# LiWentomng/OrientedRepPoints

Hardware: AMD Instinct MI355X
Metric: images/sec (1024x1024 DOTA, R-50 FPN) (higher is better)
Workload: dtype f32; 1 GPU; configs[1]: OrientedRepPoints R-50 FPN inference, 1024x1024 patch, 15 classes, bs=1/GPU, nms_pre=2000, score_thr=0.05, rnms iou_thr=0.4, max_per_img=2000; random-init weights, head biases calibrated to ~2000 dets/img; global_batch=1, parallelism=replicas x1 (image-parallel, no collective), images_in_flight_per_gpu=4

## Files before the change

include/orp_hip.h:

```cpp
#ifndef ORP_HIP_H_
#define ORP_HIP_H_

#include <stddef.h>
#include <stdint.h>

#ifdef __cplusplus
extern "C" {
#endif

#define ORP_OK 0
#define ORP_EINVAL (-1)
#define ORP_EWORKSPACE (-2)
#define ORP_ETOOBIG (-3)

const char* orp_version(void);

#define ORP_NMS_MAX_BOXES 131072
size_t orp_rnms_workspace_bytes(int n);
int orp_rnms(const float* dets, int n, float iou_thr, int flavor, int presorted, int order_out,
             int64_t* keep_out, int32_t* num_keep, void* workspace, size_t workspace_bytes, void* stream);

size_t orp_rnms_batched_workspace_bytes(int n_total, int nseg, int max_seg);
int orp_rnms_batched(const float* dets, int n_total, const int32_t* seg_offsets, int nseg, int max_seg,
                     float iou_thr, int flavor, int64_t* keep_out, int32_t* num_keep,
// ... 236 lines not shown
int orp_conv1x1_pack_weight(const float* weight, int c_out, int c_in, float* packed, void* stream);
int orp_conv1x1_multi(const orp_bias_level* levels_host, int nlevels, int batch, int c_in, int c_out,
                      const float* weight_packed, const float* bias, const float* sub, int relu, void* stream);

int orp_conv1x1_bn_act_ok(int c_in, int c_out);
int orp_conv1x1_bn_act_pays(int c_in, int c_out, int hw, int batch, int has_residual);
int orp_conv1x1_bn_act_tile(int c_in, int c_out, int hw, int batch, int* tile_channels, int* tile_positions);
int orp_conv1x1_bn_act(const float* x, const float* weight_t, const float* scale, const float* shift, const float* residual,
                       const float* scale2, const float* shift2, float* y, int batch, int c_in, int c_out, int hw, int relu,
                       void* stream);

int orp_conv1x1_bn_act_range(const float* x, const float* weight_t, const float* scale, const float* shift, const float* residual,
                             const float* scale2, const float* shift2, float* y, int batch, int c_in, int c_out, int hw, int relu,
                             uint32_t* range_out, void* stream);
int orp_conv1x1_bn_act_pieces_ok(int c_in, int c_out);
int orp_conv1x1_bn_act_pieces_pays(int c_in, int c_out, int hw, int batch, int has_residual);
int orp_conv1x1_bn_act_pieces_tile(int c_in, int c_out, int hw, int batch, int* tile_channels, int* tile_positions);
size_t orp_conv1x1_bn_pieces_packed_bytes(int c_in, int c_out);
int orp_conv1x1_bn_pieces_pack_weight(const float* weight, int c_in, int c_out, void* packed, void* stream);
int orp_conv1x1_bn_act_pieces(const float* x, const void* weight_packed, const float* scale, const float* shift,
                              const float* residual, const float* scale2, const float* shift2, float* y, int batch, int c_in,
                              int c_out, int hw, int relu, uint32_t* range_out, void* stream);

int orp_affine_act_range(const float* x, const float* residual, const float* scale, const float* shift, float* y, int batch,
                         int channels, int hw, int relu, uint32_t* range_out, void* stream);

int orp_conv3x3_bn_act_ok(int c_in, int c_out);
int orp_conv3x3_bn_act_pays(int c_in, int c_out, int height, int width, int batch);
int orp_conv3x3_bn_act_tile(int c_in, int c_out, int height, int width, int batch, int* tile_h, int* tile_w, int* waves_pos,
                            int* waves_ch);
size_t orp_conv3x3_bn_packed_bytes(int c_in, int c_out);
int orp_conv3x3_bn_pack_weight(const float* weight, int c_in, int c_out, void* packed, void* stream);
int orp_conv3x3_bn_act(const float* x, const void* weight_packed, const float* scale, const float* shift, const uint32_t* range_in,
                       float* y, int batch, int c_in, int c_out, int height, int width, int relu, void* stream);


int orp_conv3x3_small_ok(int c_in, int c_out);
int orp_conv3x3_small_multi(const orp_norm_level* levels_host, int nlevels, int batch, int c_in, int c_out,
                            const float* weight_packed, void* stream);
int orp_conv3x3_small_multi_ex(const orp_norm_level* levels_host, const float* const* weights_packed_host, int nlevels,
                               int batch, int c_in, int c_out, void* stream);
size_t orp_conv3x3_small_workspace_bytes(const orp_norm_level* levels_host, const int* strides_host, int nlevels, int batch,
                                         int c_out);
int orp_conv3x3_small_multi_strided(const orp_norm_level* levels_host, const float* const* weights_packed_host,
                                    const int* strides_host, int nlevels, int batch, int c_in, int c_out, void* workspace,
                                    size_t workspace_bytes, void* stream);
// ... 72 lines not shown
```

orientedreppoints_amd/_lib.py:

```python
import ctypes
import os

import torch

_HERE = os.path.dirname(os.path.abspath(__file__))
LIB_PATH = os.environ.get("ORP_HIP_LIB") or os.path.join(_HERE, "csrc", "liborp_hip.so")

ORP_OK, ORP_EINVAL, ORP_EWORKSPACE, ORP_ETOOBIG = 0, -1, -2, -3
ORP_NMS_MAX_BOXES = 131072

_vp = ctypes.c_void_p
_i = ctypes.c_int
_f = ctypes.c_float
_sz = ctypes.c_size_t

_SIGNATURES = {
    "orp_version": (ctypes.c_char_p, []),
    "orp_rnms_workspace_bytes": (_sz, [_i]),
    "orp_rnms": (_i, [_vp, _i, _f, _i, _i, _i, _vp, _vp, _vp, _sz, _vp]),
    "orp_rnms_batched_workspace_bytes": (_sz, [_i, _i, _i]),
    "orp_rnms_batched": (_i, [_vp, _i, _vp, _i, _i, _f, _i, _vp, _vp, _vp, _sz, _vp]),
    "_poly_nms": (None, [_vp, _vp, _vp, _i, _i, _f, _i]),
    "_overlaps": (None, [_vp, _vp, _vp, _i, _i, _i]),
    "orp_quad_iou_matrix": (_i, [_vp, _i, _vp, _i, _i, _i, _vp, _vp]),
# ... 63 lines not shown
                                     _i, _vp, _vp]),
    "orp_scene_tiles_flip": (_i, [_vp, _i, _i, ctypes.c_longlong, _vp, _i, _i, _vp, _vp, _i, _i, _vp, _vp]),
    "orp_scene_tiles_resized_flip": (_i, [_vp, _i, _i, ctypes.c_longlong, _vp, _i, _i, _i, _i, _i, _i, _i, _vp, _vp, _vp, _vp, _vp,
                                          _vp, _i, _i, _vp, _vp]),
    "orp_scene_collect_workspace_bytes": (_sz, [_i, _i]),
    "orp_scene_collect": (_i, [_vp, _i, _i, _vp, ctypes.c_double, _i, _i, _vp, _vp, _vp, _vp, _vp, _sz, _vp]),
    "orp_soft_rnms_host": (_i, [_vp, _i, _f, _i, _f, _f, _vp, _vp]),
    "orp_conv1x1_packed_floats": (_sz, [_i]),
    "orp_conv1x1_ok": (_i, [_i, _i]),
    "orp_conv1x1_pack_weight": (_i, [_vp, _i, _i, _vp, _vp]),
    "orp_conv1x1_multi": (_i, [_vp, _i, _i, _i, _i, _vp, _vp, _vp, _i, _vp]),
    "orp_conv1x1_bn_act_ok": (_i, [_i, _i]),
    "orp_conv1x1_bn_act_pays": (_i, [_i, _i, _i, _i, _i]),
    "orp_conv1x1_bn_act_tile": (_i, [_i, _i, _i, _i, _vp, _vp]),
    "orp_conv1x1_bn_act": (_i, [_vp, _vp, _vp, _vp, _vp, _vp, _vp, _vp, _i, _i, _i, _i, _i, _vp]),
    "orp_conv1x1_bn_act_range": (_i, [_vp, _vp, _vp, _vp, _vp, _vp, _vp, _vp, _i, _i, _i, _i, _i, _vp, _vp]),
    "orp_affine_act_range": (_i, [_vp, _vp, _vp, _vp, _vp, _i, _i, _i, _i, _vp, _vp]),
    "orp_conv1x1_bn_act_pieces_ok": (_i, [_i, _i]),
    "orp_conv1x1_bn_act_pieces_pays": (_i, [_i, _i, _i, _i, _i]),
    "orp_conv1x1_bn_act_pieces_tile": (_i, [_i, _i, _i, _i, _vp, _vp]),
    "orp_conv1x1_bn_pieces_packed_bytes": (_sz, [_i, _i]),
    "orp_conv1x1_bn_pieces_pack_weight": (_i, [_vp, _i, _i, _vp, _vp]),
    "orp_conv1x1_bn_act_pieces": (_i, [_vp, _vp, _vp, _vp, _vp, _vp, _vp, _vp, _i, _i, _i, _i, _i, _vp, _vp]),
    "orp_conv3x3_bn_act_ok": (_i, [_i, _i]),
    "orp_conv3x3_bn_act_pays": (_i, [_i, _i, _i, _i, _i]),
    "orp_conv3x3_bn_act_tile": (_i, [_i, _i, _i, _i, _i, _vp, _vp, _vp, _vp]),
    "orp_conv3x3_bn_packed_bytes": (_sz, [_i, _i]),
    "orp_conv3x3_bn_pack_weight": (_i, [_vp, _i, _i, _vp, _vp]),
    "orp_conv3x3_bn_act": (_i, [_vp, _vp, _vp, _vp, _vp, _vp, _i, _i, _i, _i, _i, _i, _vp]),
    "orp_pp_select_scratch_bytes": (_sz, [_i, _i, _i]),
    "orp_pp_select": (_i, [_vp, _i, _i, _vp, _i, _i, _vp, _vp, _sz, _vp]),
    "orp_pp_gather": (_i, [_vp, _vp, _i, _i, _vp, _vp, _vp, _i, _vp, _vp, _vp, _vp, _vp]),
    "orp_pp_compact_scratch_bytes": (_sz, [_i]),
    "orp_pp_compact": (_i, [_vp, _vp, _i, _i, _i, _vp, _f, _i, _vp, _vp, _vp, _vp, _vp, _vp, _sz, _vp]),
    "orp_pp_compact_views_scratch_bytes": (_sz, [_i]),
    "orp_pp_compact_views": (_i, [_vp, _i, _i, _f, _i, _vp, _vp, _vp, _vp, _vp, _vp, _vp, _vp, _sz, _vp]),
    "orp_pp_pack": (_i, [_vp, _vp, _vp, _vp, _vp, _vp, _vp, _vp, _i, _i, _vp, _vp]),
    "orp_groupnorm_workspace_bytes": (_sz, [_vp, _i, _i, _i, _i]),
    "orp_groupnorm_act_multi": (_i, [_vp, _i, _i, _i, _i, _vp, _vp, _f, _i, _vp, _sz, _vp]),
    "orp_groupnorm_act_multi_ex": (_i, [_vp, _vp, _vp, _i, _i, _i, _i, _f, _i, _vp, _sz, _vp]),
    "orp_groupnorm_act_multi_nhwc": (_i, [_vp, _vp, _vp, _vp, _i, _i, _i, _i, _f, _i, _vp, _sz, _vp]),
    "orp_groupnorm_act_multi_train": (_i, [_vp, _vp, _vp, _i, _i, _i, _i, _f, _i, _vp, _vp, _sz, _vp]),
    "orp_groupnorm_backward_workspace_bytes": (_sz, [_vp, _i, _i, _i, _i]),
    "orp_groupnorm_act_multi_backward": (_i, [_vp, _vp, _vp, _vp, _vp, _vp, _vp, _i, _i, _i, _i, _i, _vp, _vp, _sz, _vp]),
    "orp_voc_best_match_f64": (_i, [_vp, _vp, _i, _vp, _vp, _i, _vp, _vp, _vp]),
    "orp_affine_act": (_i, [_vp, _vp, _vp, _vp, _vp, _i, _i, _i, _i, _vp]),
# ... 104 lines not shown
```

orientedreppoints_amd/csrc/orp_conv1x1_bn_pieces.hip:

```cpp
#include <hip/hip_runtime.h>
#include <stdint.h>

#include "../../include/orp_hip.h"
#include "orp_affine.hpp"
#include "orp_range.hpp"
#include "orp_launch.hpp"

namespace {

constexpr int kThreads = 256;

typedef float f32x16 __attribute__((ext_vector_type(16)));
typedef __bf16 bf8 __attribute__((ext_vector_type(8)));

struct Args {
  const float* x;
  const uint16_t* planes;
  size_t plane_stride;
  const float* scale; const float* shift;
  const float* res;
  const float* scale2; const float* shift2;
  float* y;
  int cin, cout, hw, relu;
  int ntm, ntn;
  unsigned* range;
};

__global__ void pack_pieces_kernel(const float* __restrict__ w, int cout, int cin, uint16_t* __restrict__ planes) {
  const long total = (long)cout * cin;
  for (long i = (long)blockIdx.x * blockDim.x + threadIdx.x; i < total; i += (long)gridDim.x * blockDim.x) {
    const int e = (int)(i & 7);
    long r = i >> 3;
    const int o = (int)(r % cout); r /= cout;
    const int kg = (int)(r & 1);
    const int cblk = (int)(r >> 1);
    const int c = cblk * 16 + kg * 8 + e;
    const float v = w[(long)o * cin + c];
    const float v0 = __uint_as_float(__float_as_uint(v) & 0xffff0000u);
    const float r1 = v - v0;
    const float v1 = __uint_as_float(__float_as_uint(r1) & 0xffff0000u);
    const float v2 = r1 - v1;
    planes[i] = (uint16_t)(__float_as_uint(v0) >> 16);
    planes[total + i] = (uint16_t)(__float_as_uint(v1) >> 16);
    planes[2 * total + i] = (uint16_t)(__float_as_uint(v2) >> 16);
  }
}

__device__ __forceinline__ unsigned pack_hi16(float a, float b) {
  return __builtin_amdgcn_perm(__float_as_uint(b), __float_as_uint(a), 0x07060302u);
}

__device__ __forceinline__ void split_pair(float a, float b, unsigned (&d)[3]) {
  const float a0 = __uint_as_float(__float_as_uint(a) & 0xffff0000u), b0 = __uint_as_float(__float_as_uint(b) & 0xffff0000u);
  const float ar = a - a0, br = b - b0;
  const float a1 = __uint_as_float(__float_as_uint(ar) & 0xffff0000u), b1 = __uint_as_float(__float_as_uint(br) & 0xffff0000u);
  d[0] = pack_hi16(a0, b0);
  d[1] = pack_hi16(a1, b1);
  d[2] = pack_hi16(ar - a1, br - b1);
}

template <int WCH, int WN, int BK, bool VEC, int MODE, bool RANGE = false>
__global__ void __launch_bounds__(kThreads, 2)
conv1x1_bn_pieces_kernel(const Args P) {
  constexpr int ASTR = BK + 8;
  constexpr int NCH = BK / 16;
  constexpr int WPOS = 4 / WCH;
  constexpr int BM = 32 * WCH, BN = 32 * WN * WPOS;
  constexpr int PLANE = BN * ASTR, BUF = 3 * PLANE;
  constexpr int ITEMS = (BK / 2) * (BN / 4);
  constexpr int XV = (ITEMS + kThreads - 1) / kThreads;
  __shared__ __align__(16) uint16_t lds[2 * BUF + 8 * BM];
  float* Cs = reinterpret_cast<float*>(lds + 2 * BUF);

  const int tid = threadIdx.x;
  const int bid = blockIdx.x;
  const int mt = bid % P.ntm, rest = bid / P.ntm;
  const int nt = rest % P.ntn, b = rest / P.ntn;
  const int m0 = mt * BM, p0 = nt * BN;
  const int hw = P.hw, cout = P.cout;
  const float* xb = P.x + (size_t)b * P.cin * hw;
  if (tid < BM) {
    const int ch = min(m0 + tid, cout - 1);
    Cs[tid] = P.scale[ch]; Cs[BM + tid] = P.shift[ch];
    if (MODE == 2) { Cs[2 * BM + tid] = P.scale2[ch]; Cs[3 * BM + tid] = P.shift2[ch]; }
  }

  const int lane = tid & 63, wave = tid >> 6;
  const int kg = lane >> 5, l31 = lane & 31;
  const int wm0 = (wave / WPOS) * 32, wn0 = (wave % WPOS) * 32 * WN;

  const uint16_t* wp = P.planes + ((size_t)kg * cout + min(m0 + wm0 + l31, cout - 1)) * 8;
  const size_t wblk = (size_t)2 * cout * 8;
  bf8 wq[NCH][3];
  auto load_w = [&](int t, int c) {
    const uint16_t* a = wp + (size_t)(t * NCH + c) * wblk;
#pragma unroll
    for (int pl = 0; pl < 3; pl++) wq[c][pl] = *reinterpret_cast<const bf8*>(a + (size_t)pl * P.plane_stride);
  };
#pragma unroll
  for (int c = 0; c < NCH; c++) load_w(0, c);

  float4 xr[2][XV][2];
  int xpq[XV], xkp[XV];
#pragma unroll
  for (int i = 0; i < XV; i++) {
    const int idx = tid + i * kThreads;
    if (BN >= 64) {
      const int r = idx >> 5;
      xpq[i] = (idx & 15) + 16 * (r % (BN / 64));
      xkp[i] = ((idx >> 4) & 1) + 2 * (r / (BN / 64));
    } else {
      xpq[i] = idx & (BN / 4 - 1);
      xkp[i] = idx / (BN / 4);
    }
    xkp[i] &= BK / 2 - 1;
  }
  auto fetch = [&](int k0, float4 (&xr)[XV][2]) {
#pragma unroll
    for (int i = 0; i < XV; i++) {
      const int col = p0 + 4 * xpq[i];
#pragma unroll
      for (int h = 0; h < 2; h++) {
        const float* src = xb + (size_t)(k0 + 2 * xkp[i] + h) * hw;
        if (VEC) {
          xr[i][h] = *reinterpret_cast<const float4*>(src + min(col, hw - 4));
        } else {
          xr[i][h].x = src[min(col, hw - 1)]; xr[i][h].y = src[min(col + 1, hw - 1)];
          xr[i][h].z = src[min(col + 2, hw - 1)]; xr[i][h].w = src[min(col + 3, hw - 1)];
        }
      }
    }
  };
  auto stage = [&](int buf, const float4 (&xr)[XV][2]) {
#pragma unroll
    for (int i = 0; i < XV; i++) {
      if (ITEMS % kThreads != 0 && tid + i * kThreads >= ITEMS) continue;
      const int col = p0 + 4 * xpq[i];
      float v[2][4];
#pragma unroll
      for (int h = 0; h < 2; h++) {
        v[h][0] = col < hw ? xr[i][h].x : 0.f; v[h][1] = col + 1 < hw ? xr[i][h].y : 0.f;
        v[h][2] = col + 2 < hw ? xr[i][h].z : 0.f; v[h][3] = col + 3 < hw ? xr[i][h].w : 0.f;
      }
      const int rot = (xpq[i] >> 1) & 3;
#pragma unroll
      for (int h = 0; h < 2; h++) {
        if (rot & 1) { const float t0 = v[h][0]; v[h][0] = v[h][1]; v[h][1] = v[h][2]; v[h][2] = v[h][3]; v[h][3] = t0; }
        if (rot & 2) { const float t0 = v[h][0], t1 = v[h][1]; v[h][0] = v[h][2]; v[h][1] = v[h][3]; v[h][2] = t0; v[h][3] = t1; }
      }
      unsigned* base = reinterpret_cast<unsigned*>(lds + buf * BUF) + xkp[i];
#pragma unroll
      for (int j = 0; j < 4; j++) {
        unsigned d[3];
        split_pair(v[0][j], v[1][j], d);
        unsigned* dst = base + (4 * xpq[i] + ((j + rot) & 3)) * (ASTR / 2);
#pragma unroll
        for (int pl = 0; pl < 3; pl++) dst[pl * (PLANE / 2)] = d[pl];
      }
    }
  };

  f32x16 acc[WN];
#pragma unroll
  for (int ni = 0; ni < WN; ni++)
#pragma unroll
    for (int r = 0; r < 16; r++) acc[ni][r] = 0.f;

  auto mma = [&](int buf, int t_next) {
    const uint16_t* xa = lds + buf * BUF + (wn0 + l31) * ASTR + 8 * kg;
    auto load_x = [&](int c, bf8 (&q)[WN][3]) {
#pragma unroll
      for (int ni = 0; ni < WN; ni++)
#pragma unroll
        for (int pl = 0; pl < 3; pl++) q[ni][pl] = *reinterpret_cast<const bf8*>(xa + pl * PLANE + ni * 32 * ASTR + c * 16);
    };
    constexpr bool AHEAD = WN <= 2;
    bf8 xqs[AHEAD ? 2 : 1][WN][3];
    load_x(0, xqs[0]);
#pragma unroll
    for (int c = 0; c < NCH; c++) {
      bf8 (&xq)[WN][3] = xqs[AHEAD ? (c & 1) : 0];
      if (AHEAD) { if (c + 1 < NCH) load_x(c + 1, xqs[(c + 1) & 1]); }
      else if (c > 0) load_x(c, xqs[0]);
      __builtin_amdgcn_sched_barrier(0);
#pragma unroll
      for (int ni = 0; ni < WN; ni++) acc[ni] = __builtin_amdgcn_mfma_f32_32x32x16_bf16(wq[c][0], xq[ni][2], acc[ni], 0, 0, 0);
#pragma unroll
      for (int ni = 0; ni < WN; ni++) acc[ni] = __builtin_amdgcn_mfma_f32_32x32x16_bf16(wq[c][2], xq[ni][0], acc[ni], 0, 0, 0);
#pragma unroll
      for (int ni = 0; ni < WN; ni++) acc[ni] = __builtin_amdgcn_mfma_f32_32x32x16_bf16(wq[c][1], xq[ni][1], acc[ni], 0, 0, 0);
#pragma unroll
      for (int ni = 0; ni < WN; ni++) acc[ni] = __builtin_amdgcn_mfma_f32_32x32x16_bf16(wq[c][0], xq[ni][1], acc[ni], 0, 0, 0);
#pragma unroll
      for (int ni = 0; ni < WN; ni++) acc[ni] = __builtin_amdgcn_mfma_f32_32x32x16_bf16(wq[c][1], xq[ni][0], acc[ni], 0, 0, 0);
#pragma unroll
      for (int ni = 0; ni < WN; ni++) acc[ni] = __builtin_amdgcn_mfma_f32_32x32x16_bf16(wq[c][0], xq[ni][0], acc[ni], 0, 0, 0);
      __builtin_amdgcn_sched_barrier(0);
      load_w(t_next, c);
      __builtin_amdgcn_sched_barrier(0);
    }
  };

  const int nk = P.cin / BK;
  auto step = [&](int t, float4 (&cur)[XV][2], float4 (&nxt)[XV][2], int buf) {
    fetch(min(t + 2, nk - 1) * BK, cur);
    __builtin_amdgcn_sched_barrier(0);
    mma(buf, t + 1);
    stage(buf ^ 1, nxt);
    __syncthreads();
  };
  fetch(0, xr[0]);
  stage(0, xr[0]);
  fetch(min(1, nk - 1) * BK, xr[1]);
  __syncthreads();
  int t = 0;
  for (; t + 2 < nk; t += 2) {
    step(t, xr[0], xr[1], 0);
    step(t + 1, xr[1], xr[0], 1);
  }
  if (t + 1 < nk) step(t, xr[0], xr[1], 0);

  const size_t plane0 = (size_t)b * cout;
  float rv[WN][16];
  if (MODE) {
#pragma unroll
    for (int ni = 0; ni < WN; ni++) {
      const int p = min(p0 + wn0 + 32 * ni + l31, hw - 1);
#pragma unroll
      for (int r = 0; r < 16; r++) {
        const int ch = min(m0 + wm0 + 8 * (r >> 2) + 4 * kg + (r & 3), cout - 1);
        rv[ni][r] = P.res[(plane0 + ch) * hw + p];
      }
    }
  }
  __builtin_amdgcn_sched_barrier(0);
  mma((nk - 1) & 1, nk - 1);

  unsigned rmax = 0u;
#pragma unroll
  for (int g = 0; g < 4; g++) {
    const int chg = m0 + wm0 + 8 * g + 4 * kg;
    const float* cs = Cs + wm0 + 8 * g + 4 * kg;
    const float4 a4 = *reinterpret_cast<const float4*>(cs);
    const float4 b4 = *reinterpret_cast<const float4*>(cs + BM);
    const float av[4] = {a4.x, a4.y, a4.z, a4.w}, bv[4] = {b4.x, b4.y, b4.z, b4.w};
    float a2v[4] = {0.f, 0.f, 0.f, 0.f}, b2v[4] = {0.f, 0.f, 0.f, 0.f};
    if (MODE == 2) {
      const float4 c4 = *reinterpret_cast<const float4*>(cs + 2 * BM);
      const float4 d4 = *reinterpret_cast<const float4*>(cs + 3 * BM);
      a2v[0] = c4.x; a2v[1] = c4.y; a2v[2] = c4.z; a2v[3] = c4.w;
      b2v[0] = d4.x; b2v[1] = d4.y; b2v[2] = d4.z; b2v[3] = d4.w;
    }
#pragma unroll
    for (int ni = 0; ni < WN; ni++) {
      const int p = p0 + wn0 + 32 * ni + l31;
#pragma unroll
      for (int q = 0; q < 4; q++) {
        const int r = 4 * g + q;
        const float v = acc[ni][r];
        float t;
        if (MODE == 0) t = affine_act(v, av[q], bv[q], P.relu);
        else if (MODE == 1) t = affine_res_act(v, av[q], bv[q], rv[ni][r], P.relu);
        else t = affine_res_act(v, av[q], bv[q], affine_act(rv[ni][r], a2v[q], b2v[q], 0), P.relu);
        if (chg < cout && p < hw) {
          P.y[(plane0 + chg + q) * hw + p] = t;
          if (RANGE) rmax = max(rmax, orp::range_bits(t));
        }
      }
    }
  }
  if (RANGE) {
#pragma unroll
    for (int o = 32; o > 0; o >>= 1) rmax = max(rmax, (unsigned)__shfl_xor((int)rmax, o, 64));
    unsigned* red = reinterpret_cast<unsigned*>(lds);
    __syncthreads();
    if (lane == 0) red[wave] = rmax;
    __syncthreads();
    if (tid == 0) orp::range_raise(P.range, max(max(red[0], red[1]), max(red[2], red[3])));
  }
}

struct Tile { int bm, bn; };

Tile pick_tile(int cout, int hw, int batch) {
  if (cout <= 64) return Tile{64, 128};
// ... 1 lines not shown
  for (int i = 0; i < 3; i++) {
    const Tile t = cand[i];
    const long wgs = (long)((cout + t.bm - 1) / t.bm) * ((hw + t.bn - 1) / t.bn) * batch;
    if (wgs >= 512) return t;
  }
  return cand[2];
}

template <int WCH, int WN, int BK, int MODE>
void launch_mode(const Args& A, int batch, bool vec, hipStream_t st) {
  const dim3 grid((unsigned)((long)A.ntm * A.ntn * batch));
  if (vec) hipLaunchKernelGGL((conv1x1_bn_pieces_kernel<WCH, WN, BK, true, MODE>), grid, dim3(kThreads), 0, st, A);
  else hipLaunchKernelGGL((conv1x1_bn_pieces_kernel<WCH, WN, BK, false, MODE>), grid, dim3(kThreads), 0, st, A);
}
template <int WCH, int WN, int BK>
void launch(const Args& A, int batch, bool vec, hipStream_t st) {
  if (A.range) {
    const dim3 grid((unsigned)((long)A.ntm * A.ntn * batch));
    if (vec) hipLaunchKernelGGL((conv1x1_bn_pieces_kernel<WCH, WN, BK, true, 0, true>), grid, dim3(kThreads), 0, st, A);
    else hipLaunchKernelGGL((conv1x1_bn_pieces_kernel<WCH, WN, BK, false, 0, true>), grid, dim3(kThreads), 0, st, A);
  } else if (!A.res) launch_mode<WCH, WN, BK, 0>(A, batch, vec, st);
  else if (!A.scale2) launch_mode<WCH, WN, BK, 1>(A, batch, vec, st);
  else launch_mode<WCH, WN, BK, 2>(A, batch, vec, st);
}

}

extern "C" {

int orp_conv1x1_bn_act_pieces_ok(int c_in, int c_out) {
  return (c_in >= 64 && c_in <= 2048 && c_in % 64 == 0 && c_out >= 64 && c_out <= 4096 && c_out % 32 == 0) ? 1 : 0;
}

int orp_conv1x1_bn_act_pieces_tile(int c_in, int c_out, int hw, int batch, int* tile_channels, int* tile_positions) {
  if (!orp_conv1x1_bn_act_pieces_ok(c_in, c_out) || hw <= 0 || batch <= 0) return 0;
  const Tile t = pick_tile(c_out, hw, batch);
  if (tile_channels) *tile_channels = t.bm;
  if (tile_positions) *tile_positions = t.bn;
  return 1;
}

int orp_conv1x1_bn_act_pieces_pays(int c_in, int c_out, int hw, int batch, int has_residual) {
  if (!orp_conv1x1_bn_act_pieces_ok(c_in, c_out) || hw <= 0 || batch <= 0) return 0;
  (void)has_residual;
  static const struct { int cin, cout, hw_min, hw_max, batch; } paid[] = {
      {64, 64, 65536, 65536, 1},
      {256, 64, 65536, 147456, 1},  {256, 64, 65536, 65536, 2},
      {64, 256, 65536, 147456, 1},  {64, 256, 65536, 65536, 2},
      {256, 128, 65536, 147456, 1}, {256, 128, 65536, 65536, 2},
      {512, 128, 16384, 36864, 1},  {512, 128, 16384, 16384, 2},
      {128, 512, 16384, 36864, 1},  {128, 512, 16384, 16384, 2},
      {512, 256, 16384, 36864, 1},  {512, 256, 16384, 16384, 2},
      {1024, 256, 4096, 9216, 1},   {1024, 256, 4096, 4096, 2},
      {256, 1024, 4096, 9216, 1},   {256, 1024, 4096, 4096, 2},
      {1024, 512, 4096, 9216, 1},   {1024, 512, 4096, 4096, 2},
      {2048, 512, 2304, 2304, 1},   {2048, 512, 1024, 1024, 2},
      {512, 2048, 1024, 2304, 1},   {512, 2048, 1024, 1024, 2},
  };
  for (const auto& s : paid)
    if (s.cin == c_in && s.cout == c_out && s.batch == batch && hw >= s.hw_min && hw <= s.hw_max) return 1;
  return 0;
}

size_t orp_conv1x1_bn_pieces_packed_bytes(int c_in, int c_out) {
  return orp_conv1x1_bn_act_pieces_ok(c_in, c_out) ? (size_t)6 * c_in * c_out : 0;
}

int orp_conv1x1_bn_pieces_pack_weight(const float* weight, int c_in, int c_out, void* packed, void* stream) {
  if (!weight || !packed || ((uintptr_t)packed & 15) || !orp_conv1x1_bn_act_pieces_ok(c_in, c_out)) return ORP_EINVAL;
  const long total = (long)c_in * c_out;
  const int blocks = (int)((total + 255) / 256 < 4096 ? (total + 255) / 256 : 4096);
  hipLaunchKernelGGL(pack_pieces_kernel, dim3(blocks), dim3(256), 0, (hipStream_t)stream, weight, c_out, c_in,
                     reinterpret_cast<uint16_t*>(packed));
  hipError_t e = hipGetLastError();
  return e == hipSuccess ? ORP_OK : (int)e;
}

int orp_conv1x1_bn_act_pieces(const float* x, const void* weight_packed, const float* scale, const float* shift, const float* residual,
                              const float* scale2, const float* shift2, float* y, int batch, int c_in, int c_out, int hw, int relu,
                              uint32_t* range_out, void* stream) {
  if (range_out && residual) return ORP_EINVAL;
  if (!x || !weight_packed || !scale || !shift || !y || batch <= 0 || hw <= 0 || !orp_conv1x1_bn_act_pieces_ok(c_in, c_out))
    return ORP_EINVAL;
// ... 2 lines not shown
  if ((uintptr_t)weight_packed & 15) return ORP_EINVAL;
  const Tile t = pick_tile(c_out, hw, batch);
  Args A;
  A.x = x; A.planes = reinterpret_cast<const uint16_t*>(weight_packed); A.plane_stride = (size_t)c_in * c_out;
  A.scale = scale; A.shift = shift; A.res = residual; A.scale2 = scale2; A.shift2 = shift2; A.y = y;
  A.cin = c_in; A.cout = c_out; A.hw = hw; A.relu = relu ? 1 : 0;
  A.ntm = (c_out + t.bm - 1) / t.bm; A.ntn = (hw + t.bn - 1) / t.bn;
  A.range = range_out;
  if ((long)A.ntm * A.ntn * batch >= (1L << 31)) return ORP_ETOOBIG;
  const bool vec = (hw & 3) == 0 && ((uintptr_t)x & 15) == 0;
  hipStream_t st = (hipStream_t)stream;
  if (range_out) {
    hipError_t fe = orp::fill_async(range_out, 0, sizeof(uint32_t), st);
    if (fe != hipSuccess) return (int)fe;
  }
  if (t.bm == 64) launch<2, 2, 32>(A, batch, vec, st);
  else if (t.bn == 128) launch<4, 4, 32>(A, batch, vec, st);
  else if (t.bn == 64) launch<4, 2, 64>(A, batch, vec, st);
  else launch<4, 1, 64>(A, batch, vec, st);
  hipError_t e = hipGetLastError();
  return e == hipSuccess ? ORP_OK : (int)e;
}

}
```

orientedreppoints_amd/mmdet_models/resnet.py:

```python
import torch
import torch.nn as nn

from .layers import build_conv_layer, build_norm_layer, constant_init, kaiming_init
from .registry import BACKBONES


class Bottleneck(nn.Module):
    expansion = 4

    def __init__(self, inplanes, planes, stride=1, dilation=1, downsample=None, style='pytorch',
                 norm_cfg=dict(type='BN'), dcn=None):
        super(Bottleneck, self).__init__()
        assert style in ['pytorch', 'caffe']
        assert dcn is None or isinstance(dcn, dict)
        if style == 'pytorch':
            conv1_stride, conv2_stride = 1, stride
        else:
            conv1_stride, conv2_stride = stride, 1
        self.conv1 = nn.Conv2d(inplanes, planes, kernel_size=1, stride=conv1_stride, bias=False)
        self.add_module('bn1', build_norm_layer(norm_cfg, planes)[1])
        self.with_dcn = dcn is not None
        fallback_on_stride = False
        if self.with_dcn:
            fallback_on_stride = dcn.pop('fallback_on_stride', False)
            dcn = dict(dcn)
            if 'modulated' in dcn:
                dcn.setdefault('type', 'DCNv2' if dcn.pop('modulated') else 'DCN')
            dcn.setdefault('type', 'DCN')
        use_dcn = self.with_dcn and not fallback_on_stride
        self.conv2 = build_conv_layer(dcn if use_dcn else None, planes, planes, kernel_size=3, stride=conv2_stride,
                                      padding=dilation, dilation=dilation, bias=False)
        self.conv2_is_dcn = use_dcn
        self.add_module('bn2', build_norm_layer(norm_cfg, planes)[1])
        self.conv3 = nn.Conv2d(planes, planes * self.expansion, kernel_size=1, bias=False)
        self.add_module('bn3', build_norm_layer(norm_cfg, planes * self.expansion)[1])
        self.relu = nn.ReLU(inplace=True)
        self.downsample = downsample

    def _fused_ok(self, x):
        return (not torch.is_grad_enabled()) and x.is_cuda and x.dtype == torch.float32 and \
            isinstance(self.bn1, nn.BatchNorm2d) and not self.bn1.training and not self.bn3.training

    def _downsample_norm_fusable(self):
        from .. import switches
        on = getattr(self, 'fuse_downsample_norm', None)
        if on is None:
            on = switches.BN_DOWNSAMPLE_FUSE
        ds = self.downsample
        return bool(on) and isinstance(ds, nn.Sequential) and len(ds) == 2 and isinstance(ds[0], nn.Conv2d) and \
            isinstance(ds[1], nn.BatchNorm2d) and not ds[1].training

    def _conv1x1_fusable(self):
        from .. import switches
        on = getattr(self, 'fuse_conv1x1', None)
        if on is None:
            on = switches.BN_CONV1X1_FUSE
        return bool(on)

    def _conv1x1_pieces_on(self):
        from .. import switches
        on = getattr(self, 'fuse_conv1x1_pieces', None)
        if on is None:
            on = switches.BN_CONV1X1_PIECES
        return bool(on)

    def _conv3x3_fusable(self):
        from .. import switches
        on = getattr(self, 'fuse_conv3x3', None)
        if on is None:
            on = switches.BN_CONV3X3_FUSE
        return bool(on) and not self.conv2_is_dcn and isinstance(self.bn2, nn.BatchNorm2d) and not self.bn2.training

    def _forward_fused(self, x):
        from ..mmdet_ops.fused_norm import bn_act, conv1x1_bn_act, conv3x3_bn_act, conv3x3_bn_act_routed
        fuse = self._conv1x1_fusable()
        pieces = None if self._conv1x1_pieces_on() else False

        def conv_bn_act(t, conv, bn, **kw):
            if fuse:
                return conv1x1_bn_act(t, conv, bn, pieces=pieces, **kw)
            return bn_act(conv(t).contiguous(), bn, **kw)
        force3 = bool(getattr(self, 'force_conv3x3', False))
        fuse3 = False
        if self._conv3x3_fusable() and tuple(self.conv1.stride) == (1, 1):
            fuse3 = conv3x3_bn_act_routed(x, self.conv2, self.bn2, force3,
                                          shape=(x.size(0), self.conv1.out_channels, x.size(2), x.size(3)))
        if fuse3:
            out, bits = conv_bn_act(x, self.conv1, self.bn1, relu=True, want_range=True)
            out = conv3x3_bn_act(out, self.conv2, self.bn2, relu=True, force=force3, range_bits=bits)
        else:
            out = conv_bn_act(x, self.conv1, self.bn1, relu=True)
            out = bn_act(self.conv2(out).contiguous(), self.bn2, relu=True)
        if self._downsample_norm_fusable():
            return conv_bn_act(out, self.conv3, self.bn3, residual=self.downsample[0](x).contiguous(),
                               residual_bn=self.downsample[1], relu=True)
        if self.downsample is not None:
            identity = bn_act(self.downsample[0](x).contiguous(), self.downsample[1], relu=False)
        else:
            identity = x.contiguous()
        return conv_bn_act(out, self.conv3, self.bn3, residual=identity, relu=True)

    def forward(self, x):
        if self._fused_ok(x):
            return self._forward_fused(x)
        identity = x
        out = self.relu(self.bn1(self.conv1(x)))
        out = self.relu(self.bn2(self.conv2(out)))
        out = self.bn3(self.conv3(out))
        if self.downsample is not None:
            identity = self.downsample(x)
        out += identity
        return self.relu(out)


@BACKBONES.register_module
# ... 130 lines not shown
```

orientedreppoints_amd/mmdet_ops/fused_norm.py:

```python
import ctypes

import torch

from .. import _lib, _packcache


class _NormLevel(ctypes.Structure):
    _fields_ = [("input", ctypes.c_void_p), ("output", ctypes.c_void_p), ("height", ctypes.c_int),
                ("width", ctypes.c_int)]


def _norm_levels(ins, outs):
    levels = (_NormLevel * len(ins))()
    for i, (x, y) in enumerate(zip(ins, outs)):
        levels[i] = _NormLevel(x.data_ptr(), y.data_ptr() if y is not None else None, x.size(2), x.size(3))
    return levels


def _gn_modules(gn, n, who):
    gns = list(gn) if isinstance(gn, (list, tuple)) else [gn] * n
    if len(gns) != n or any(g.num_groups != gns[0].num_groups or g.eps != gns[0].eps for g in gns):
        raise ValueError(who + ": one GroupNorm per tensor, equal num_groups / eps")
    index, distinct, owner = {}, [], []
    for g in gns:
# ... 232 lines not shown
    if residual is not None:
        residual = residual.detach()
        if not (tuple(residual.shape) == (B, cout, H, W) and residual.is_contiguous() and residual.dtype == torch.float32):
            raise ValueError("conv1x1_bn_act: residual must be a contiguous fp32 tensor of the output's shape")
    wt = _transposed_1x1_weight(conv.weight)
    scale, shift = _bn_affine(bn)
    scale2, shift2 = _bn_affine(residual_bn) if residual_bn is not None else (None, None)
    y = torch.empty((B, cout, H, W), dtype=torch.float32, device=x.device)
    if want_range:
        bits = torch.empty(1, dtype=torch.int32, device=x.device)
        with torch.cuda.device(x.device):
            rc = L.orp_conv1x1_bn_act_range(_lib.ptr(x), _lib.ptr(wt), _lib.ptr(scale), _lib.ptr(shift), None, None, None,
                                            _lib.ptr(y), B, cin, cout, H * W, 1 if relu else 0, _lib.ptr(bits), _lib.stream_of(x))
        _lib.check(rc, "orp_conv1x1_bn_act_range")
        return y, bits
    with torch.cuda.device(x.device):
        rc = L.orp_conv1x1_bn_act(_lib.ptr(x), _lib.ptr(wt), _lib.ptr(scale), _lib.ptr(shift), _lib.ptr(residual),
                                  _lib.ptr(scale2), _lib.ptr(shift2), _lib.ptr(y), B, cin, cout, H * W, 1 if relu else 0,
                                  _lib.stream_of(x))
    _lib.check(rc, "orp_conv1x1_bn_act")
    return y


def conv3x3_bn_act_ok(x, conv, bn, shape=None):
    w = getattr(conv, 'weight', None)
    shape = tuple(x.shape) if shape is None else tuple(shape)
    return bool(type(conv) is torch.nn.Conv2d and isinstance(bn, torch.nn.BatchNorm2d) and not bn.training and
                x.is_cuda and x.dtype == torch.float32 and len(shape) == 4 and w.dtype == torch.float32 and w.dim() == 4 and
                w.size(2) == 3 and w.size(3) == 3 and shape[1] == w.size(1) and conv.bias is None and
                tuple(conv.stride) == (1, 1) and tuple(conv.padding) == (1, 1) and tuple(conv.dilation) == (1, 1) and
                conv.groups == 1 and shape[0] * shape[2] * shape[3] > 0 and _lib.lib().orp_conv3x3_bn_act_ok(w.size(1), w.size(0)))


def conv3x3_bn_act_routed(x, conv, bn, force=False, shape=None):
    if not conv3x3_bn_act_ok(x, conv, bn, shape):
        return False
    B, _c, H, W = tuple(x.shape) if shape is None else tuple(shape)
    return bool(force or _lib.lib().orp_conv3x3_bn_act_pays(conv.weight.size(1), conv.weight.size(0), H, W, B))


def conv3x3_bn_act_tile(cin, cout, H, W, B):
    v = [ctypes.c_int() for _ in range(4)]
    if not _lib.lib().orp_conv3x3_bn_act_tile(int(cin), int(cout), int(H), int(W), int(B), *[ctypes.byref(t) for t in v]):
        return None
    return tuple(t.value for t in v)

# ... 690 lines not shown
```

orientedreppoints_amd/switches.py:

```python
import os


def _on(name, default='1'):
    return os.environ.get(name, default) == '1'


TOWER_SPLIT = _on('ORP_TOWER_SPLIT')
FPN_SPLIT = _on('ORP_FPN_SPLIT')
TOWER_GN_FUSE = _on('ORP_TOWER_GN_FUSE')
BN_DOWNSAMPLE_FUSE = _on('ORP_BN_DOWNSAMPLE_FUSE')
BN_CONV1X1_FUSE = _on('ORP_BN_CONV1X1_FUSE')
BN_CONV1X1_PIECES = _on('ORP_BN_CONV1X1_PIECES')
BN_CONV3X3_FUSE = _on('ORP_BN_CONV3X3_FUSE')
STEM_POOL_FUSE = _on('ORP_STEM_POOL_FUSE')
FPN_TOPDOWN_FUSE = _on('ORP_FPN_TOPDOWN_FUSE')
TRAIN_SPLIT = _on('ORP_TRAIN_SPLIT')
DETERMINISTIC = _on('ORP_DETERMINISTIC', '0')
```

Before: 433.3 images/s.

## Fuse ResNet downsample 1x1 conv into conv3 bottleneck pieces kernel

Adds a dual-input mode to the bf16-pieces 1x1 conv kernel. It first accumulates the downsample branch (optionally stride-2 sampled from the block input), applies its BN affine into registers, then computes conv3 with BN plus that residual and ReLU. This removes the separate downsample conv launch and the write and read of its intermediate tensor in the first block of each ResNet stage. It is gated by a table of shapes where it is expected to pay, and it adds kernel complexity plus strided, non-coalesced loads for the stride-2 branch.

```diff
diff --git a/include/orp_hip.h b/include/orp_hip.h
--- a/include/orp_hip.h
+++ b/include/orp_hip.h
@@ -282,6 +282,13 @@
                               const float* residual, const float* scale2, const float* shift2, float* y, int batch, int c_in,
                               int c_out, int hw, int relu, uint32_t* range_out, void* stream);
 
+int orp_conv1x1_bn_act_pieces_dual_ok(int c_in, int c_in2, int c_out);
+int orp_conv1x1_bn_act_pieces_dual_pays(int c_in, int c_in2, int c_out, int hw, int stride2, int batch);
+int orp_conv1x1_bn_act_pieces_dual_tile(int c_in, int c_in2, int c_out, int hw, int batch, int* tile_channels, int* tile_positions);
+int orp_conv1x1_bn_act_pieces_dual(const float* x, const void* w_packed, const float* scale, const float* shift, const float* x2,
+                                   const void* w2_packed, const float* scale2, const float* shift2, int c_in2, int h2, int w2,
+                                   int stride2, float* y, int batch, int c_in, int c_out, int ho, int wo, int relu, void* stream);
+
 int orp_affine_act_range(const float* x, const float* residual, const float* scale, const float* shift, float* y, int batch,
                          int channels, int hw, int relu, uint32_t* range_out, void* stream);
 
diff --git a/orientedreppoints_amd/_lib.py b/orientedreppoints_amd/_lib.py
--- a/orientedreppoints_amd/_lib.py
+++ b/orientedreppoints_amd/_lib.py
@@ -109,6 +109,10 @@
     "orp_conv1x1_bn_pieces_packed_bytes": (_sz, [_i, _i]),
     "orp_conv1x1_bn_pieces_pack_weight": (_i, [_vp, _i, _i, _vp, _vp]),
     "orp_conv1x1_bn_act_pieces": (_i, [_vp, _vp, _vp, _vp, _vp, _vp, _vp, _vp, _i, _i, _i, _i, _i, _vp, _vp]),
+    "orp_conv1x1_bn_act_pieces_dual_ok": (_i, [_i, _i, _i]),
+    "orp_conv1x1_bn_act_pieces_dual_pays": (_i, [_i, _i, _i, _i, _i, _i]),
+    "orp_conv1x1_bn_act_pieces_dual_tile": (_i, [_i, _i, _i, _i, _i, _vp, _vp]),
+    "orp_conv1x1_bn_act_pieces_dual": (_i, [_vp, _vp, _vp, _vp, _vp, _vp, _vp, _vp, _i, _i, _i, _i, _vp, _i, _i, _i, _i, _i, _i, _vp]),
     "orp_conv3x3_bn_act_ok": (_i, [_i, _i]),
     "orp_conv3x3_bn_act_pays": (_i, [_i, _i, _i, _i, _i]),
     "orp_conv3x3_bn_act_tile": (_i, [_i, _i, _i, _i, _i, _vp, _vp, _vp, _vp]),
diff --git a/orientedreppoints_amd/csrc/orp_conv1x1_bn_pieces.hip b/orientedreppoints_amd/csrc/orp_conv1x1_bn_pieces.hip
--- a/orientedreppoints_amd/csrc/orp_conv1x1_bn_pieces.hip
+++ b/orientedreppoints_amd/csrc/orp_conv1x1_bn_pieces.hip
@@ -1,5 +1,6 @@
 #include <hip/hip_runtime.h>
 #include <stdint.h>
+#include <type_traits>
 
 #include "../../include/orp_hip.h"
 #include "orp_affine.hpp"
@@ -24,6 +25,12 @@
   int cin, cout, hw, relu;
   int ntm, ntn;
   unsigned* range;
+};
+struct DualArgs : Args {
+  const float* x2;
+  const uint16_t* planes2;
+  size_t plane_stride2;
+  int cin2, hw2, w2, wo, s2;
 };
 
 __global__ void pack_pieces_kernel(const float* __restrict__ w, int cout, int cin, uint16_t* __restrict__ planes) {
@@ -59,9 +66,9 @@
   d[2] = pack_hi16(ar - a1, br - b1);
 }
 
-template <int WCH, int WN, int BK, bool VEC, int MODE, bool RANGE = false>
+template <int WCH, int WN, int BK, bool VEC, int MODE, bool RANGE = false, bool SAMP = false>
 __global__ void __launch_bounds__(kThreads, 2)
-conv1x1_bn_pieces_kernel(const Args P) {
+conv1x1_bn_pieces_kernel(const typename std::conditional<MODE == 3, DualArgs, Args>::type P) {
   constexpr int ASTR = BK + 8;
   constexpr int NCH = BK / 16;
   constexpr int WPOS = 4 / WCH;
@@ -82,7 +89,7 @@
   if (tid < BM) {
     const int ch = min(m0 + tid, cout - 1);
     Cs[tid] = P.scale[ch]; Cs[BM + tid] = P.shift[ch];
-    if (MODE == 2) { Cs[2 * BM + tid] = P.scale2[ch]; Cs[3 * BM + tid] = P.shift2[ch]; }
+    if (MODE >= 2) { Cs[2 * BM + tid] = P.scale2[ch]; Cs[3 * BM + tid] = P.shift2[ch]; }
   }
 
   const int lane = tid & 63, wave = tid >> 6;
@@ -90,15 +97,20 @@
   const int wm0 = (wave / WPOS) * 32, wn0 = (wave % WPOS) * 32 * WN;
 
   const uint16_t* wp = P.planes + ((size_t)kg * cout + min(m0 + wm0 + l31, cout - 1)) * 8;
+  const uint16_t* wp2 = nullptr;
+  size_t ps2 = 0;
+  if constexpr (MODE == 3) ps2 = P.plane_stride2;
+  if constexpr (MODE == 3) wp2 = P.planes2 + ((size_t)kg * cout + min(m0 + wm0 + l31, cout - 1)) * 8;
   const size_t wblk = (size_t)2 * cout * 8;
   bf8 wq[NCH][3];
-  auto load_w = [&](int t, int c) {
-    const uint16_t* a = wp + (size_t)(t * NCH + c) * wblk;
-#pragma unroll
-    for (int pl = 0; pl < 3; pl++) wq[c][pl] = *reinterpret_cast<const bf8*>(a + (size_t)pl * P.plane_stride);
-  };
-#pragma unroll
-  for (int c = 0; c < NCH; c++) load_w(0, c);
+  auto load_w = [&](bool br, int t, int c) {
+    const uint16_t* a = (br ? wp2 : wp) + (size_t)(t * NCH + c) * wblk;
+    const size_t ps = br ? ps2 : P.plane_stride;
+#pragma unroll
+    for (int pl = 0; pl < 3; pl++) wq[c][pl] = *reinterpret_cast<const bf8*>(a + (size_t)pl * ps);
+  };
+#pragma unroll
+  for (int c = 0; c < NCH; c++) load_w(MODE == 3, 0, c);
 
   float4 xr[2][XV][2];
   int xpq[XV], xkp[XV];
@@ -115,6 +127,41 @@
     }
     xkp[i] &= BK / 2 - 1;
   }
+  constexpr int NXO = MODE == 3 ? (VEC ? 1 : 4) : 0;
+  int xo[XV][NXO > 0 ? NXO : 1];
+  const float* x2b = nullptr;
+  if constexpr (MODE == 3) {
+    x2b = P.x2 + (size_t)b * P.cin2 * P.hw2;
+#pragma unroll
+    for (int i = 0; i < XV; i++) {
+      const int col = p0 + 4 * xpq[i];
+#pragma unroll
+      for (int j = 0; j < NXO; j++) {
+        const int p = VEC ? min(col, hw - 4) : min(col + j, hw - 1);
+        const int oy = p / P.wo;
+        xo[i][j] = P.s2 * (oy * P.w2 + (p - oy * P.wo));
+      }
+    }
+  }
+  auto fetch2 = [&](int k0, float4 (&xr)[XV][2]) {
+    if constexpr (MODE == 3)
+#pragma unroll
+    for (int i = 0; i < XV; i++) {
+#pragma unroll
+      for (int h = 0; h < 2; h++) {
+        const float* src = x2b + (size_t)(k0 + 2 * xkp[i] + h) * P.hw2;
+        if (VEC && !SAMP) {
+          xr[i][h] = *reinterpret_cast<const float4*>(src + xo[i][0]);
+        } else if (VEC) {
+          const float* q = src + xo[i][0];
+          xr[i][h].x = q[0]; xr[i][h].y = q[2]; xr[i][h].z = q[4]; xr[i][h].w = q[6];
+        } else {
+          xr[i][h].x = src[xo[i][0]]; xr[i][h].y = src[xo[i][NXO > 1 ? 1 : 0]];
+          xr[i][h].z = src[xo[i][NXO > 1 ? 2 : 0]]; xr[i][h].w = src[xo[i][NXO > 1 ? 3 : 0]];
+        }
+      }
+    }
+  };
   auto fetch = [&](int k0, float4 (&xr)[XV][2]) {
 #pragma unroll
     for (int i = 0; i < XV; i++) {
@@ -124,6 +171,11 @@
         const float* src = xb + (size_t)(k0 + 2 * xkp[i] + h) * hw;
         if (VEC) {
           xr[i][h] = *reinterpret_cast<const float4*>(src + min(col, hw - 4));
+        } else if (MODE == 3) {
+          int o[4];
+#pragma unroll
+          for (int j = 0; j < 4; j++) { o[j] = min(col + j, hw - 1); asm volatile("" : "+v"(o[j])); }
+          xr[i][h].x = src[o[0]]; xr[i][h].y = src[o[1]]; xr[i][h].z = src[o[2]]; xr[i][h].w = src[o[3]];
         } else {
           xr[i][h].x = src[min(col, hw - 1)]; xr[i][h].y = src[min(col + 1, hw - 1)];
           xr[i][h].z = src[min(col + 2, hw - 1)]; xr[i][h].w = src[min(col + 3, hw - 1)];
@@ -166,7 +218,7 @@
 #pragma unroll
     for (int r = 0; r < 16; r++) acc[ni][r] = 0.f;
 
-  auto mma = [&](int buf, int t_next) {
+  auto mma = [&](bool wnext, int buf, int t_next) {
     const uint16_t* xa = lds + buf * BUF + (wn0 + l31) * ASTR + 8 * kg;
     auto load_x = [&](int c, bf8 (&q)[WN][3]) {
 #pragma unroll
@@ -174,7 +226,7 @@
 #pragma unroll
         for (int pl = 0; pl < 3; pl++) q[ni][pl] = *reinterpret_cast<const bf8*>(xa + pl * PLANE + ni * 32 * ASTR + c * 16);
     };
-    constexpr bool AHEAD = WN <= 2;
+    constexpr bool AHEAD = WN <= 2 && !(MODE == 3 && WN == 2);
     bf8 xqs[AHEAD ? 2 : 1][WN][3];
     load_x(0, xqs[0]);
 #pragma unroll
@@ -196,33 +248,68 @@
 #pragma unroll
       for (int ni = 0; ni < WN; ni++) acc[ni] = __builtin_amdgcn_mfma_f32_32x32x16_bf16(wq[c][0], xq[ni][0], acc[ni], 0, 0, 0);
       __builtin_amdgcn_sched_barrier(0);
-      load_w(t_next, c);
+      load_w(wnext, t_next, c);
       __builtin_amdgcn_sched_barrier(0);
     }
   };
 
   const int nk = P.cin / BK;
-  auto step = [&](int t, float4 (&cur)[XV][2], float4 (&nxt)[XV][2], int buf) {
-    fetch(min(t + 2, nk - 1) * BK, cur);
+  auto step = [&](bool br, int nk, int t, float4 (&cur)[XV][2], float4 (&nxt)[XV][2], int buf) {
+    if (MODE == 3 && br) fetch2(min(t + 2, nk - 1) * BK, cur);
+    else fetch(min(t + 2, nk - 1) * BK, cur);
     __builtin_amdgcn_sched_barrier(0);
-    mma(buf, t + 1);
+    mma(br, buf, t + 1);
     stage(buf ^ 1, nxt);
     __syncthreads();
   };
-  fetch(0, xr[0]);
-  stage(0, xr[0]);
-  fetch(min(1, nk - 1) * BK, xr[1]);
+  float rv[WN][16];
+  if constexpr (MODE == 3) {
+    const int nk2 = P.cin2 / BK;
+    fetch2(0, xr[0]);
+    stage(0, xr[0]);
+    fetch2(min(1, nk2 - 1) * BK, xr[1]);
+    __syncthreads();
+    int t = 0;
+    for (; t + 2 < nk2; t += 2) {
+      step(true, nk2, t, xr[0], xr[1], 0);
+      step(true, nk2, t + 1, xr[1], xr[0], 1);
+    }
+    if (t + 1 < nk2) step(true, nk2, t, xr[0], xr[1], 0);
+    fetch(0, xr[0]);
+    fetch(min(1, nk - 1) * BK, xr[1]);
+    __builtin_amdgcn_sched_barrier(0);
+    mma(false, (nk2 - 1) & 1, 0);
+#pragma unroll
+    for (int g = 0; g < 4; g++) {
+      const float* cs = Cs + wm0 + 8 * g + 4 * kg;
+      const float4 c4 = *reinterpret_cast<const float4*>(cs + 2 * BM);
+      const float4 d4 = *reinterpret_cast<const float4*>(cs + 3 * BM);
+      const float a2v[4] = {c4.x, c4.y, c4.z, c4.w}, b2v[4] = {d4.x, d4.y, d4.z, d4.w};
+#pragma unroll
+      for (int ni = 0; ni < WN; ni++)
+#pragma unroll
+        for (int q = 0; q < 4; q++) {
+          rv[ni][4 * g + q] = affine_act(acc[ni][4 * g + q], a2v[q], b2v[q], 0);
+          acc[ni][4 * g + q] = 0.f;
+        }
+    }
+    __syncthreads();
+    stage(0, xr[0]);
+  } else {
+    fetch(0, xr[0]);
+    stage(0, xr[0]);
+    fetch(min(1, nk - 1) * BK, xr[1]);
+  }
   __syncthreads();
   int t = 0;
   for (; t + 2 < nk; t += 2) {
-    step(t, xr[0], xr[1], 0);
-    step(t + 1, xr[1], xr[0], 1);
-  }
-  if (t + 1 < nk) step(t, xr[0], xr[1], 0);
+    step(false, nk, t, xr[0], xr[1], 0);
+    step(false, nk, t + 1, xr[1], xr[0], 1);
+  }
+  if (t + 1 < nk) step(false, nk, t, xr[0], xr[1], 0);
 
   const size_t plane0 = (size_t)b * cout;
-  float rv[WN][16];
-  if (MODE) {
+  if (MODE == 1 || MODE == 2) {
 #pragma unroll
     for (int ni = 0; ni < WN; ni++) {
       const int p = min(p0 + wn0 + 32 * ni + l31, hw - 1);
@@ -234,7 +321,7 @@
     }
   }
   __builtin_amdgcn_sched_barrier(0);
-  mma((nk - 1) & 1, nk - 1);
+  mma(false, (nk - 1) & 1, nk - 1);
 
   unsigned rmax = 0u;
 #pragma unroll
@@ -260,7 +347,7 @@
         const float v = acc[ni][r];
         float t;
         if (MODE == 0) t = affine_act(v, av[q], bv[q], P.relu);
-        else if (MODE == 1) t = affine_res_act(v, av[q], bv[q], rv[ni][r], P.relu);
+        else if (MODE == 1 || MODE == 3) t = affine_res_act(v, av[q], bv[q], rv[ni][r], P.relu);
         else t = affine_res_act(v, av[q], bv[q], affine_act(rv[ni][r], a2v[q], b2v[q], 0), P.relu);
         if (chg < cout && p < hw) {
           P.y[(plane0 + chg + q) * hw + p] = t;
@@ -308,6 +395,19 @@
   } else if (!A.res) launch_mode<WCH, WN, BK, 0>(A, batch, vec, st);
   else if (!A.scale2) launch_mode<WCH, WN, BK, 1>(A, batch, vec, st);
   else launch_mode<WCH, WN, BK, 2>(A, batch, vec, st);
+}
+
+Tile pick_tile_dual(int cout, int hw, int batch) {
+  const long wgs = (long)((cout + 127) / 128) * ((hw + 63) / 64) * batch;
+  return wgs >= 512 ? Tile{128, 64} : Tile{128, 32};
+}
+
+template <int WN>
+void launch_dual(const DualArgs& A, int batch, bool vec, hipStream_t st) {
+  const dim3 grid((unsigned)((long)A.ntm * A.ntn * batch));
+  if (vec && A.s2 == 1) hipLaunchKernelGGL((conv1x1_bn_pieces_kernel<4, WN, 64, true, 3, false, false>), grid, dim3(kThreads), 0, st, A);
+  else if (vec) hipLaunchKernelGGL((conv1x1_bn_pieces_kernel<4, WN, 64, true, 3, false, true>), grid, dim3(kThreads), 0, st, A);
+  else hipLaunchKernelGGL((conv1x1_bn_pieces_kernel<4, WN, 64, false, 3, false, true>), grid, dim3(kThreads), 0, st, A);
 }
 
 }
@@ -345,6 +445,33 @@
   };
   for (const auto& s : paid)
     if (s.cin == c_in && s.cout == c_out && s.batch == batch && hw >= s.hw_min && hw <= s.hw_max) return 1;
+  return 0;
+}
+
+int orp_conv1x1_bn_act_pieces_dual_ok(int c_in, int c_in2, int c_out) {
+  return (orp_conv1x1_bn_act_pieces_ok(c_in, c_out) && orp_conv1x1_bn_act_pieces_ok(c_in2, c_out)) ? 1 : 0;
+}
+
+int orp_conv1x1_bn_act_pieces_dual_tile(int c_in, int c_in2, int c_out, int hw, int batch, int* tile_channels, int* tile_positions) {
+  if (!orp_conv1x1_bn_act_pieces_dual_ok(c_in, c_in2, c_out) || hw <= 0 || batch <= 0) return 0;
+  const Tile t = pick_tile_dual(c_out, hw, batch);
+  if (tile_channels) *tile_channels = t.bm;
+  if (tile_positions) *tile_positions = t.bn;
+  return 1;
+}
+
+int orp_conv1x1_bn_act_pieces_dual_pays(int c_in, int c_in2, int c_out, int hw, int stride2, int batch) {
+  if (!orp_conv1x1_bn_act_pieces_dual_ok(c_in, c_in2, c_out) || hw <= 0 || batch <= 0) return 0;
+  if (!orp_conv1x1_bn_act_pieces_pays(c_in, c_out, hw, batch, 1)) return 0;
+  static const struct { int cin, cin2, cout, stride, hw_min, hw_max, batch; } paid[] = {
+      {64, 64, 256, 1, 65536, 147456, 1},    {64, 64, 256, 1, 65536, 65536, 2},
+      {128, 256, 512, 2, 16384, 36864, 1},   {128, 256, 512, 2, 16384, 16384, 2},
+      {256, 512, 1024, 2, 4096, 9216, 1},    {256, 512, 1024, 2, 4096, 4096, 2},
+  };
+  for (const auto& s : paid)
+    if (s.cin == c_in && s.cin2 == c_in2 && s.cout == c_out && s.stride == stride2 && s.batch == batch && hw >= s.hw_min &&
+        hw <= s.hw_max)
+      return 1;
   return 0;
 }
 
@@ -393,4 +520,34 @@
   return e == hipSuccess ? ORP_OK : (int)e;
 }
 
-}
+int orp_conv1x1_bn_act_pieces_dual(const float* x, const void* w_packed, const float* scale, const float* shift, const float* x2,
+                                   const void* w2_packed, const float* scale2, const float* shift2, int c_in2, int h2, int w2,
+                                   int stride2, float* y, int batch, int c_in, int c_out, int ho, int wo, int relu, void* stream) {
+  if (!x || !w_packed || !scale || !shift || !x2 || !w2_packed || !scale2 || !shift2 || !y || batch <= 0 || ho <= 0 || wo <= 0 ||
+      h2 <= 0 || w2 <= 0 || !orp_conv1x1_bn_act_pieces_dual_ok(c_in, c_in2, c_out))
+    return ORP_EINVAL;
+  if (stride2 != 1 && stride2 != 2) return ORP_EINVAL;
+  if (ho != (h2 - 1) / stride2 + 1 || wo != (w2 - 1) / stride2 + 1) return ORP_EINVAL;
+  if ((const float*)y == x || (const float*)y == x2) return ORP_EINVAL;
+  if (((uintptr_t)w_packed & 15) || ((uintptr_t)w2_packed & 15)) return ORP_EINVAL;
+  if ((long)ho * wo >= (1L << 31) / 4 || (long)h2 * w2 >= (1L << 31) / 4) return ORP_ETOOBIG;
+  const int hw = ho * wo;
+  const Tile t = pick_tile_dual(c_out, hw, batch);
+  DualArgs A{};
+  A.x = x; A.planes = reinterpret_cast<const uint16_t*>(w_packed); A.plane_stride = (size_t)c_in * c_out;
+  A.scale = scale; A.shift = shift; A.res = nullptr; A.scale2 = scale2; A.shift2 = shift2; A.y = y;
+  A.cin = c_in; A.cout = c_out; A.hw = hw; A.relu = relu ? 1 : 0;
+  A.ntm = (c_out + t.bm - 1) / t.bm; A.ntn = (hw + t.bn - 1) / t.bn;
+  A.range = nullptr;
+  A.x2 = x2; A.planes2 = reinterpret_cast<const uint16_t*>(w2_packed); A.plane_stride2 = (size_t)c_in2 * c_out;
+  A.cin2 = c_in2; A.hw2 = h2 * w2; A.w2 = w2; A.wo = wo; A.s2 = stride2;
+  if ((long)A.ntm * A.ntn * batch >= (1L << 31)) return ORP_ETOOBIG;
+  const bool vec = (hw & 3) == 0 && ((uintptr_t)x & 15) == 0 && ((uintptr_t)x2 & 15) == 0 && (stride2 == 1 || (wo & 3) == 0);
+  hipStream_t st = (hipStream_t)stream;
+  if (t.bn == 64) launch_dual<2>(A, batch, vec, st);
+  else launch_dual<1>(A, batch, vec, st);
+  hipError_t e = hipGetLastError();
+  return e == hipSuccess ? ORP_OK : (int)e;
+}
+
+}
diff --git a/orientedreppoints_amd/mmdet_models/resnet.py b/orientedreppoints_amd/mmdet_models/resnet.py
--- a/orientedreppoints_amd/mmdet_models/resnet.py
+++ b/orientedreppoints_amd/mmdet_models/resnet.py
@@ -46,8 +46,11 @@
         on = getattr(self, 'fuse_downsample_norm', None)
         if on is None:
             on = switches.BN_DOWNSAMPLE_FUSE
+        return bool(on) and self._downsample_is_conv_norm()
+
+    def _downsample_is_conv_norm(self):
         ds = self.downsample
-        return bool(on) and isinstance(ds, nn.Sequential) and len(ds) == 2 and isinstance(ds[0], nn.Conv2d) and \
+        return isinstance(ds, nn.Sequential) and len(ds) == 2 and isinstance(ds[0], nn.Conv2d) and \
             isinstance(ds[1], nn.BatchNorm2d) and not ds[1].training
 
     def _conv1x1_fusable(self):
@@ -64,6 +67,13 @@
             on = switches.BN_CONV1X1_PIECES
         return bool(on)
 
+    def _downsample_conv_fusable(self):
+        from .. import switches
+        on = getattr(self, 'fuse_downsample_conv', None)
+        if on is None:
+            on = switches.BN_DOWNSAMPLE_CONV_FUSE
+        return bool(on)
+
     def _conv3x3_fusable(self):
         from .. import switches
         on = getattr(self, 'fuse_conv3x3', None)
@@ -72,7 +82,8 @@
         return bool(on) and not self.conv2_is_dcn and isinstance(self.bn2, nn.BatchNorm2d) and not self.bn2.training
 
     def _forward_fused(self, x):
-        from ..mmdet_ops.fused_norm import bn_act, conv1x1_bn_act, conv3x3_bn_act, conv3x3_bn_act_routed
+        from ..mmdet_ops.fused_norm import bn_act, conv1x1_bn_act, conv3x3_bn_act, conv3x3_bn_act_routed, \
+            conv1x1_bn_act_dual, conv1x1_bn_act_dual_ok, conv1x1_bn_act_dual_pays
         fuse = self._conv1x1_fusable()
         pieces = None if self._conv1x1_pieces_on() else False
 
@@ -91,6 +102,11 @@
         else:
             out = conv_bn_act(x, self.conv1, self.bn1, relu=True)
             out = bn_act(self.conv2(out).contiguous(), self.bn2, relu=True)
+        ds = self.downsample
+        if fuse and pieces is None and self._downsample_conv_fusable() and self._downsample_is_conv_norm() and \
+                conv1x1_bn_act_dual_ok(out, self.conv3, self.bn3, x, ds[0], ds[1]) and \
+                conv1x1_bn_act_dual_pays(out, self.conv3, x, ds[0]):
+            return conv1x1_bn_act_dual(out, self.conv3, self.bn3, x, ds[0], ds[1], relu=True)
         if self._downsample_norm_fusable():
             return conv_bn_act(out, self.conv3, self.bn3, residual=self.downsample[0](x).contiguous(),
                                residual_bn=self.downsample[1], relu=True)
diff --git a/orientedreppoints_amd/mmdet_ops/fused_norm.py b/orientedreppoints_amd/mmdet_ops/fused_norm.py
--- a/orientedreppoints_amd/mmdet_ops/fused_norm.py
+++ b/orientedreppoints_amd/mmdet_ops/fused_norm.py
@@ -278,6 +278,52 @@
     return y
 
 
+def conv1x1_bn_act_dual_ok(x, conv, bn, x2, conv2, bn2):
+    if not conv1x1_bn_act_ok(x, conv, bn):
+        return False
+    w2 = getattr(conv2, 'weight', None)
+    if not (isinstance(conv2, torch.nn.Conv2d) and isinstance(bn2, torch.nn.BatchNorm2d) and not bn2.training and
+            x2.is_cuda and x2.dtype == torch.float32 and x2.dim() == 4 and x2.device == x.device and w2.dtype == torch.float32 and
+            w2.dim() == 4 and w2.size(2) == 1 and w2.size(3) == 1 and x2.size(1) == w2.size(1) and conv2.bias is None and
+            tuple(conv2.stride) in ((1, 1), (2, 2)) and tuple(conv2.padding) == (0, 0) and tuple(conv2.dilation) == (1, 1) and
+            conv2.groups == 1 and w2.size(0) == conv.weight.size(0) and x2.size(0) == x.size(0)):
+        return False
+    s = conv2.stride[0]
+    return bool(x2.size(2) > 0 and x2.size(3) > 0 and (x2.size(2) - 1) // s + 1 == x.size(2) and (x2.size(3) - 1) // s + 1 == x.size(3)
+                and _lib.lib().orp_conv1x1_bn_act_pieces_dual_ok(conv.weight.size(1), w2.size(1), w2.size(0)))
+
+
+def conv1x1_bn_act_dual_pays(x, conv, x2, conv2):
+    return bool(_lib.lib().orp_conv1x1_bn_act_pieces_dual_pays(conv.weight.size(1), conv2.weight.size(1), conv.weight.size(0),
+                                                               x.size(2) * x.size(3), conv2.stride[0], x.size(0)))
+
+
+def conv1x1_bn_act_dual_tile(cin, cin2, cout, hw, B):
+    v = [ctypes.c_int() for _ in range(2)]
+    if not _lib.lib().orp_conv1x1_bn_act_pieces_dual_tile(int(cin), int(cin2), int(cout), int(hw), int(B), *[ctypes.byref(t) for t in v]):
+        return None
+    return tuple(t.value for t in v)
+
+
+def conv1x1_bn_act_dual(x, conv, bn, x2, conv2, bn2, relu=True):
+    if not conv1x1_bn_act_dual_ok(x, conv, bn, x2, conv2, bn2):
+        raise ValueError("conv1x1_bn_act_dual: unsupported modules or shapes (conv1x1_bn_act_dual_ok)")
+    L = _lib.lib()
+    x, x2 = x.detach().contiguous(), x2.detach().contiguous()
+    B, cin, H, W = x.shape
+    cout, cin2 = conv.weight.size(0), conv2.weight.size(1)
+    packed, packed2 = _packed_1x1_planes(conv.weight), _packed_1x1_planes(conv2.weight)
+    scale, shift = _bn_affine(bn)
+    scale2, shift2 = _bn_affine(bn2)
+    y = torch.empty((B, cout, H, W), dtype=torch.float32, device=x.device)
+    with torch.cuda.device(x.device):
+        rc = L.orp_conv1x1_bn_act_pieces_dual(_lib.ptr(x), _lib.ptr(packed), _lib.ptr(scale), _lib.ptr(shift), _lib.ptr(x2),
+                                              _lib.ptr(packed2), _lib.ptr(scale2), _lib.ptr(shift2), cin2, x2.size(2), x2.size(3),
+                                              conv2.stride[0], _lib.ptr(y), B, cin, cout, H, W, 1 if relu else 0, _lib.stream_of(x))
+    _lib.check(rc, "orp_conv1x1_bn_act_pieces_dual")
+    return y
+
+
 def conv3x3_bn_act_ok(x, conv, bn, shape=None):
     w = getattr(conv, 'weight', None)
     shape = tuple(x.shape) if shape is None else tuple(shape)
diff --git a/orientedreppoints_amd/switches.py b/orientedreppoints_amd/switches.py
--- a/orientedreppoints_amd/switches.py
+++ b/orientedreppoints_amd/switches.py
@@ -11,6 +11,7 @@
 BN_DOWNSAMPLE_FUSE = _on('ORP_BN_DOWNSAMPLE_FUSE')
 BN_CONV1X1_FUSE = _on('ORP_BN_CONV1X1_FUSE')
 BN_CONV1X1_PIECES = _on('ORP_BN_CONV1X1_PIECES')
+BN_DOWNSAMPLE_CONV_FUSE = _on('ORP_BN_DOWNSAMPLE_CONV_FUSE')
 BN_CONV3X3_FUSE = _on('ORP_BN_CONV3X3_FUSE')
 STEM_POOL_FUSE = _on('ORP_STEM_POOL_FUSE')
 FPN_TOPDOWN_FUSE = _on('ORP_FPN_TOPDOWN_FUSE')
```

After: 440.8 images/s, median of 6. +1.7%, better.
